# linjieli222/HERO

Measured on AMD Instinct MI355X. Metric: videos/sec training step, HERO-base TVR-shaped batch, higher is better.
Workload: dtype bf16; 1 GPU; configs[1]: HERO-base TVR finetune micro-step (train-tvr-8gpu.json shapes: 32 videos x 60 frames, 15 subs x (4 frames + 20 tokens), 15-token query; vfeat 4352; fwd + VSM loss + bwd, all-reduce/clip/AdamW every 2nd micro-step); global_batch=32, parallelism=dp1, grad_accum=2, launch=hipGraph replay, input=one batch resident in HBM

## Files before the change

hero_amd/_lib.py:

```python
import ctypes as C
import os

import torch

_HERE = os.path.dirname(os.path.abspath(__file__))
LIB_PATH = os.environ.get("HERO_HIP_LIB") or os.path.join(_HERE, "libhero_hip.so")

ABI_VERSION = 3
F32, BF16 = 0, 1
LAYOUT_K, LAYOUT_O = 0, 1
ACT_NONE, ACT_GELU, ACT_RELU, ACT_GELU_BWD, ACT_RELU_BWD, ACT_GELU_DG, ACT_MUL_AUX = 0, 1, 2, 3, 4, 5, 6

EXPORTS = [
    "hero_last_error", "hero_abi_version", "hero_abi_struct_count", "hero_abi_struct_bytes", "hero_gemm", "hero_gemm_splits", "hero_fold_slabs", "hero_wgrad_group", "hero_wgrad_batch_plan", "hero_wgrad_batch", "hero_prof_enable", "hero_prof_read", "hero_probe_mfma", "hero_probe_hbm", "hero_gemm_force_config", "hero_layernorm_fwd",
    "hero_layernorm_bwd_workspace_bytes", "hero_layernorm_bwd", "hero_colsum_workspace_bytes",
    "hero_colsum", "hero_colsum_multi", "hero_colsum_multi_workspace_bytes", "hero_layernorm_bwd_blocks", "hero_attention_fwd", "hero_attention_bwd", "hero_attention_max_len", "hero_attention_max_packed_len", "hero_attention_stats_ok", "hero_attention_force_ppw",
    "hero_gather_rows", "hero_inverse_first", "hero_csr_gather_sum", "hero_scatter_add_rows", "hero_segment_sort_workspace_bytes", "hero_scatter_add_sorted_workspace_bytes", "hero_segment_sort", "hero_scatter_add_sorted", "hero_cast", "hero_transpose_cast", "hero_copy_multi",
    "hero_relu_bwd", "hero_gelu_bwd", "hero_add", "hero_sumsq", "hero_adamw", "hero_adamw_multi", "hero_adamw_multi_chunk",
    "hero_query_pool_fwd", "hero_query_pool_bwd", "hero_rownorm_fwd", "hero_rownorm_bwd", "hero_score_max_fwd",
    "hero_score_max_bwd", "hero_rank_loss", "hero_sums_scaled", "hero_st_ed_fwd", "hero_st_ed_bwd", "hero_st_ed_bwd_workspace_bytes",
    "hero_cross_entropy_fwd", "hero_cross_entropy_bwd",
    "hero_collate_subs", "hero_collate_clip_mask", "hero_collate_frame_map", "hero_collate_gather_feats", "hero_derive_multi",
    "hero_comm_available", "hero_comm_unique_id", "hero_comm_init", "hero_comm_destroy", "hero_comm_rank", "hero_comm_world",
    "hero_comm_allreduce_buckets", "hero_comm_broadcast", "hero_comm_allgather", "hero_comm_allgather_var",
]


class Dropout(C.Structure):
    _fields_ = [("seed_ptr", C.c_void_p), ("site", C.c_uint64),
                ("threshold16", C.c_uint32), ("scale", C.c_float)]


class GemmEpilogue(C.Structure):
    _fields_ = [("bias", C.c_void_p), ("residual", C.c_void_p), ("aux", C.c_void_p),
                ("act", C.c_int), ("out_f32", C.c_int), ("beta", C.c_float),
                ("split_k", C.c_int), ("dropout", Dropout), ("colsum", C.c_void_p), ("colsum_partial", C.c_int), ("pad_", C.c_int), ("split_stride", C.c_longlong)]


class CrossEntropy(C.Structure):
    _fields_ = [("logits", C.c_void_p), ("labels", C.c_void_p), ("loss", C.c_void_p), ("lse", C.c_void_p),
                ("dloss", C.c_void_p), ("dlogits", C.c_void_p), ("rows", C.c_int), ("cols", C.c_int),
                ("ld", C.c_int), ("dtype", C.c_int), ("inv_temp", C.c_float), ("ignore_index", C.c_int64)]


class Derive(C.Structure):
    _fields_ = [("src", C.c_void_p), ("dst", C.c_void_p), ("n", C.c_int64), ("mode", C.c_int), ("p0", C.c_int),
                ("p1", C.c_int), ("p2", C.c_int)]
# ... 121 lines not shown
    global _lib
    if _lib is None:
        if not os.path.exists(LIB_PATH):
            raise RuntimeError(
                "hero_amd: %s is missing. Build it with `python -m hero_amd.build` "
                "(needs hipcc; cross-compiles for gfx950 without a GPU). There is no fallback "
                "path." % LIB_PATH)
        L = C.CDLL(LIB_PATH)
        L.hero_last_error.restype = C.c_char_p
        have = L.hero_abi_version()
        if have != ABI_VERSION:
            raise RuntimeError("hero_amd: %s reports ABI version %d, this binding was written against %d (struct layouts "
                               "differ: rebuild with `python -m hero_amd.build --force`)" % (LIB_PATH, have, ABI_VERSION))
        L.hero_abi_struct_bytes.argtypes = [C.c_int]
        if L.hero_abi_struct_count() != len(ABI_STRUCTS):
            raise RuntimeError("hero_amd: %s declares %d ABI structs, this binding mirrors %d" % (LIB_PATH, L.hero_abi_struct_count(), len(ABI_STRUCTS)))
        bad = [(st.__name__, C.sizeof(st), L.hero_abi_struct_bytes(i)) for i, st in enumerate(ABI_STRUCTS)
               if C.sizeof(st) != L.hero_abi_struct_bytes(i)]
        if bad:
            raise RuntimeError("hero_amd: struct layouts differ from %s (name, binding bytes, library bytes): %s" % (LIB_PATH, bad))
        L.hero_layernorm_bwd_workspace_bytes.restype = C.c_size_t
        L.hero_colsum_workspace_bytes.restype = C.c_size_t
        L.hero_colsum_multi_workspace_bytes.restype = C.c_size_t
        L.hero_colsum_multi_workspace_bytes.argtypes = [C.POINTER(Colsum), C.c_int]
        L.hero_colsum_multi.argtypes = [C.POINTER(Colsum), C.c_int, C.c_void_p, C.c_void_p]
        L.hero_layernorm_bwd_blocks.argtypes = [C.c_int]
        L.hero_gemm.argtypes = [C.c_void_p, C.c_void_p, C.c_void_p] + [C.c_int] * 9 + [
            C.POINTER(GemmEpilogue), C.c_void_p]
        L.hero_gemm_splits.argtypes = [C.c_int, C.c_int, C.c_int]
        L.hero_fold_slabs.argtypes = [C.c_void_p, C.c_int, C.c_size_t, C.c_void_p, C.c_size_t, C.c_int, C.c_void_p]
        L.hero_wgrad_group.argtypes = [C.POINTER(WgradProblem), C.c_int, C.c_int, C.c_int, C.c_void_p]
        L.hero_wgrad_batch_plan.argtypes = [C.POINTER(WgradProblem), C.c_int, C.c_int, C.c_void_p, C.c_int]
        L.hero_wgrad_batch.argtypes = [C.POINTER(WgradProblem), C.c_int, C.c_int, C.c_int, C.c_void_p, C.c_int, C.c_void_p]
        L.hero_prof_enable.argtypes = [C.c_int]
        L.hero_prof_read.argtypes = [C.c_int, C.POINTER(C.c_double), C.POINTER(C.c_double),
                                     C.POINTER(C.c_longlong)]
        L.hero_probe_mfma.argtypes = [C.c_void_p, C.c_size_t, C.POINTER(C.c_double), C.POINTER(C.c_double), C.c_void_p]
        L.hero_probe_hbm.argtypes = [C.c_void_p, C.c_void_p, C.c_size_t, C.POINTER(C.c_double), C.POINTER(C.c_double), C.c_void_p]
        L.hero_layernorm_fwd.argtypes = [C.POINTER(LnFwd), C.c_void_p]
        L.hero_layernorm_bwd.argtypes = [C.POINTER(LnBwd), C.c_void_p]
        L.hero_layernorm_bwd_workspace_bytes.argtypes = [C.c_int, C.c_int]
        L.hero_colsum_workspace_bytes.argtypes = [C.c_int, C.c_int]
        L.hero_colsum.argtypes = [C.c_void_p, C.c_void_p, C.c_int, C.c_int, C.c_int, C.c_int,
                                  C.c_float, C.c_void_p, C.c_void_p]
        L.hero_attention_fwd.argtypes = [C.POINTER(Attn), C.c_void_p]
        L.hero_attention_bwd.argtypes = [C.POINTER(Attn), C.c_void_p]
        L.hero_attention_stats_ok.argtypes = [C.c_int, C.c_int]
        L.hero_attention_force_ppw.argtypes = [C.c_int]
        L.hero_attention_max_len.argtypes = [C.c_int, C.c_int]
        L.hero_attention_max_packed_len.argtypes = [C.c_int]
        L.hero_gather_rows.argtypes = [C.c_void_p, C.c_void_p, C.c_void_p, C.c_void_p,
                                       C.c_int, C.c_int, C.c_int, C.c_void_p]
        L.hero_inverse_first.argtypes = [C.c_void_p, C.c_int, C.c_void_p, C.c_int, C.c_int, C.c_void_p]
        L.hero_csr_gather_sum.argtypes = [C.c_void_p, C.c_void_p, C.c_void_p, C.c_void_p,
                                          C.c_int, C.c_int, C.c_int, C.c_void_p]
        L.hero_scatter_add_rows.argtypes = [C.c_void_p, C.c_void_p, C.c_void_p, C.c_void_p,
                                            C.c_int, C.c_int, C.c_int, C.c_int, C.c_int, C.c_void_p]
        L.hero_segment_sort_workspace_bytes.argtypes = [C.c_int]
        L.hero_segment_sort_workspace_bytes.restype = C.c_size_t
        L.hero_segment_sort.argtypes = [C.c_void_p, C.c_int, C.c_int, C.c_int, C.c_void_p, C.c_void_p, C.c_void_p]
        L.hero_scatter_add_sorted_workspace_bytes.argtypes = [C.c_int, C.c_int]
        L.hero_scatter_add_sorted_workspace_bytes.restype = C.c_size_t
        L.hero_scatter_add_sorted.argtypes = [C.c_void_p, C.c_void_p, C.c_void_p, C.c_void_p, C.c_int, C.c_int, C.c_int, C.c_int,
                                              C.c_void_p, C.c_void_p]
        L.hero_st_ed_bwd_workspace_bytes.argtypes = [C.c_int]
        L.hero_st_ed_bwd_workspace_bytes.restype = C.c_size_t
# ... 74 lines not shown
```

hero_amd/csrc/gemm_ws.hip:

```cpp
#include <stdlib.h>
#include <type_traits>

#include "gemm_ws_common.h"

namespace hero {
namespace ws {

template <int TM, int TN, bool TR, int EK>
__global__ __launch_bounds__(512) __attribute__((amdgpu_waves_per_eu(2, 2))) void gemm_ws_kernel(WsArgs g) {
  typedef Geo<TM, TN> G;
  extern __shared__ __attribute__((aligned(16))) char smem[];
  const int lane = threadIdx.x & 63;
  const int wave = __builtin_amdgcn_readfirstlane(threadIdx.x >> 6);
  const int nwg = gridDim.x;
  int wg;
  {
    const int bid = blockIdx.x, q = nwg >> 3, r = nwg & 7, xcd = bid & 7, loc = bid >> 3;
    wg = (xcd < r ? xcd * (q + 1) : r * (q + 1) + (xcd - r) * q) + loc;
  }

  if (wave >= 4) {
    Loader<G, TR> ld(g, smem, wg, nwg, wave - 4, lane);
    constexpr int AHEAD = (G::NSG - 2) * G::PW;
    bool more = ld.issue();
#pragma unroll
    for (int k = 0; k < G::NSG - 2; ++k) more = ld.issue();
    if (more) wait_vm<AHEAD>(); else wait_vm<0>();
    __builtin_amdgcn_s_barrier();
    unsigned slot = 0;
    int item_no = 0;
    for (int cit = wg; cit < g.nwork; cit += nwg, ++item_no) {
      const Item ic = item_coord<G>(g, cit);
      WS_T(item_no, 0, wave, lane);
// ... 351 lines not shown
      __builtin_amdgcn_s_barrier();
      __builtin_amdgcn_sched_barrier(0);
      ldf(a0, b0, nxt, 0);
      mma(a1, b1);
      WS_INTERLEAVE(TM * TN, 2 * (TM + TN));
      __builtin_amdgcn_sched_barrier(0);
    }
    pos += sg.nk;
    WS_T(seg_no, 1, wave, lane);
#ifdef HERO_WS_TRACE
    if (blockIdx.x == 0 && lane == 0 && seg_no < 4) g_ws_trace[(seg_no * 16 + 3) * 8 + wave] = (unsigned long long)sg.nk;
#endif
    const WsgProb& P = g.p[sg.prob];
#pragma unroll
    for (int i = 0; i < TM; ++i)
#pragma unroll
      for (int j = 0; j < TN; ++j) {
        const int gn = sg.n0 + brow0 + j * 32 + (lane & 31);
#pragma unroll
        for (int r = 0; r < 16; ++r) {
          const int gm = sg.m0 + arow0 + i * 32 + (r & 3) + 8 * (r >> 2) + 4 * (lane >> 5);
          if (gm < P.M && gn < P.N) atomicAdd(P.C + (size_t)gm * P.ldc + gn, acc[i][j][r]);
        }
      }
    WS_T(seg_no, 14, wave, lane);
  }
}

struct WsbProb {
  const bf16_t* A;
  const bf16_t* B;
  float* C;
  float* colsum;
  int M, N, lda, ldb, ldc, pad_;
};
struct WsbItem { int prob, m0, n0, k0, nk, order, nslices, flag; };
struct WsbArgs {
  const WsbItem* items;
  int* flags;
  int rounds, K, nprob, pad_;
  WsbProb p[HERO_WGRAD_BATCH_MAX];
};

template <typename G, bool COMPUTE>
__device__ __forceinline__ void epilogue_acc(const WsbProb& P, const WsbItem& it, int* flags, char* smem, unsigned slot,
                                             f32x16_t (*acc)[G::TN], int wave, int lane, bool want_cs = false) {
  constexpr int TM = G::TM, TN = G::TN, BN = G::BN, RPP = G::RPP, C8 = G::C8, RPI = G::RPI, ITERS = G::ITERS;
  char* st = smem + slot;
  int tid = threadIdx.x;
  asm volatile("" : "+v"(tid));
  lane = tid & 63;
  wave = __builtin_amdgcn_readfirstlane(tid >> 6);
  const int c8 = tid % C8, r0 = tid / C8;
  const int gn = it.n0 + c8 * 8;
  const bool col_ok = r0 < RPI && gn < P.N;
  const int wm = wave >> 1, wn = wave & 1, l31 = lane & 31, half = lane >> 5;
  const bool plain = it.nslices == 1;
  constexpr bool SPLIT = (RPP == 64 && G::PASSES == TM);
  auto tile_row = [](int p, int row) { return SPLIT ? (row >> 5) * (TM * 32) + p * 32 + (row & 31) : p * RPP + row; };
  const __amdgpu_buffer_rsrc_t rc = __builtin_amdgcn_make_buffer_rsrc(P.C, 0, 0x7ffffff0, 0x00020000);
  if (!plain && it.order > 0) {
    if (lane == 0)
      while (__hip_atomic_load(flags + it.flag, __ATOMIC_RELAXED, __HIP_MEMORY_SCOPE_AGENT) != it.order) __builtin_amdgcn_s_sleep(8);
  }
#pragma unroll
  for (int p = 0; p < G::PASSES; ++p) {
    u32x4_t old0[ITERS], old1[ITERS];
    unsigned voff[ITERS];
    if (plain) {
#pragma unroll
      for (int i = 0; i < ITERS; ++i) {
        const int row = r0 + i * RPI;
        const int gm = it.m0 + tile_row(p, row);
        const bool ok = col_ok && row < RPP && gm < P.M;
// ... 98 lines not shown
    wg = (xcd < r ? xcd * (q + 1) : r * (q + 1) + (xcd - r) * q) + loc;
  }
  auto next_round = [&](int r) {
    while (r < g.rounds && g.items[(size_t)r * nwg + wg].nk == 0) ++r;
    return r;
  };

  if (wave >= 4) {
    const int w = wave - 4;
    constexpr int CA = G::BM / 8, CB = G::BN / 8;
    int lr = next_round(0), ik = 0, lnk = 0;
    unsigned goa[G::PA], gob[G::PB];
    const char* pa = nullptr;
    const char* pb = nullptr;
    unsigned long long ra_left = 0, rb_left = 0;
    unsigned sa = 0, sb = 0, fill = 0;
    auto setup = [&]() {
      const WsbItem it = g.items[(size_t)lr * nwg + wg];
      const WsbProb& P = g.p[it.prob];
      lnk = it.nk;
#pragma unroll
      for (int i = 0; i < G::PA; ++i) {
        const int id = (w * G::PA + i) * 64 + lane, row = id / CA, c = (id % CA) ^ swz_o<G::BM * 2>(row);
        goa[i] = (unsigned)row * (unsigned)P.lda * 2u + (c << 4);
      }
#pragma unroll
      for (int i = 0; i < G::PB; ++i) {
        const int id = (w * G::PB + i) * 64 + lane, row = id / CB, c = (id % CB) ^ swz_o<G::BN * 2>(row);
        gob[i] = (unsigned)row * (unsigned)P.ldb * 2u + (c << 4);
      }
      const int kb = it.k0 * 64;
      pa = reinterpret_cast<const char*>(P.A + (size_t)kb * P.lda + it.m0);
      pb = reinterpret_cast<const char*>(P.B + (size_t)kb * P.ldb + it.n0);
      ra_left = ((unsigned long long)(g.K - kb) * P.lda - it.m0) * 2;
      rb_left = ((unsigned long long)(g.K - kb) * P.ldb - it.n0) * 2;
      sa = 64u * (unsigned)P.lda * 2u;
      sb = 64u * (unsigned)P.ldb * 2u;
    };
    if (lr < g.rounds) setup();
    auto issue = [&]() -> bool {
      if (lr >= g.rounds) return false;
      char* buf = smem + fill;
      const __amdgpu_buffer_rsrc_t ra = __builtin_amdgcn_make_buffer_rsrc(const_cast<char*>(pa), 0, (unsigned)(ra_left < 0xfffffff0ull ? ra_left : 0xfffffff0ull), 0x00020000);
      const __amdgpu_buffer_rsrc_t rb = __builtin_amdgcn_make_buffer_rsrc(const_cast<char*>(pb), 0, (unsigned)(rb_left < 0xfffffff0ull ? rb_left : 0xfffffff0ull), 0x00020000);
#ifndef HERO_WSB_NOLOADS
#pragma unroll
      for (int i = 0; i < G::PA; ++i)
        __builtin_amdgcn_raw_ptr_buffer_load_lds(ra, HERO_LDS_PTR(buf + (w * G::PA + i) * 1024), 16, goa[i], 0, 0, HERO_WS_LOAD_AUX_A);
#pragma unroll
      for (int i = 0; i < G::PB; ++i)
        __builtin_amdgcn_raw_ptr_buffer_load_lds(rb, HERO_LDS_PTR(buf + G::A_BYTES + (w * G::PB + i) * 1024), 16, gob[i], 0, 0, HERO_WS_LOAD_AUX_B);
#else
      (void)ra; (void)rb; (void)buf;
#endif
      fill += G::STAGE;
      if (fill == NS * G::STAGE) fill = 0;
      if (++ik == lnk) {
        ik = 0;
        lr = next_round(lr + 1);
        if (lr < g.rounds) setup();
      } else {
        pa += sa; pb += sb;
        ra_left = ra_left > sa ? ra_left - sa : 0ull;
        rb_left = rb_left > sb ? rb_left - sb : 0ull;
      }
      return true;
    };
    issue();
// ... 324 lines not shown
    P.M = q.M; P.N = q.N; P.lda = q.ld_dy; P.ldb = q.ld_x; P.ldc = q.ld_dw;
    P.tiles_n = (q.N + G::BN - 1) / G::BN;
    P.tile0 = tiles;
    tiles += ((q.M + G::BM - 1) / G::BM) * P.tiles_n;
  }
  const int ksteps = (K + 63) / 64;
  const int cus = num_cus();
  if (ok && (long long)tiles * ksteps >= 8LL * cus) {
    for (int i = n; i < 4; ++i) g.p[i] = g.p[0];
    g.nprob = n; g.K = K; g.ksteps = ksteps; g.total_tiles = tiles;
    HERO_ENSURE_LDS(&gemm_wsg_kernel, G::LDS, "gemm_wsg_kernel");
    double flops = 0.0;
    for (int i = 0; i < n; ++i) flops += 2.0 * probs[i].M * (double)probs[i].N * K;
    void* tok = gemm_prof_begin(9, s);
    hipLaunchKernelGGL(gemm_wsg_kernel, dim3(cus), dim3(512), G::LDS, s, g);
    gemm_prof_end(tok, flops, s);
    return check_launch("hero_wgrad_group");
  }
  for (int i = 0; i < n; ++i) {
    const HeroWgradProblem& q = probs[i];
    HeroGemmEpilogue e = {};
    e.out_f32 = 1; e.beta = 1.f; e.split_k = q.split_hint > 0 ? q.split_hint : 1; e.dropout.scale = 1.f;
    const int rc = hero_gemm(q.dy, q.x, q.dw, q.M, q.N, K, q.ld_dy, q.ld_x, q.ld_dw, HERO_LAYOUT_O, HERO_LAYOUT_O, dtype, &e, stream);
    if (rc) return rc;
  }
  return HERO_OK;
}

namespace hero {
namespace ws {
__device__ int g_wsb_flags[512];
constexpr int PLAN_MAGIC = 0x57534232;
constexpr int PLAN_HDR = 8;
}
}

extern "C" int hero_wgrad_batch_plan(const HeroWgradProblem* probs, int n, int K, int32_t* plan, int capacity_words) {
  using namespace hero;
  using namespace hero::ws;
  typedef Geo<3, 3> G;
  HERO_REQUIRE(probs && n >= 1 && n <= HERO_WGRAD_BATCH_MAX, "hero_wgrad_batch_plan: 1..%d problems", HERO_WGRAD_BATCH_MAX);
  HERO_REQUIRE(K >= 1, "hero_wgrad_batch_plan: K = %d", K);
  const int nwg = num_cus(), ksteps = (K + 63) / 64;
  if (nwg % 8 != 0 || ksteps < 8) return 0;
  struct T3 { int prob, mt, nt; };
  std::vector<T3> tiles;
  for (int i = 0; i < n; ++i) {
    HERO_REQUIRE(probs[i].M > 0 && probs[i].N > 0 && probs[i].M % 8 == 0 && probs[i].N % 8 == 0, "hero_wgrad_batch_plan: bad problem %d", i);
    const int tm = (probs[i].M + G::BM - 1) / G::BM, tn = (probs[i].N + G::BN - 1) / G::BN;
    const int per = nwg / 8;
    int pm = tm < 8 ? tm : 8;
    int pn = per / pm > 0 ? per / pm : 1;
    if (pn > tn) { pn = tn; pm = per / pn < tm ? per / pn : tm; if (pm < 1) pm = 1; }
    for (int bm = 0; bm < tm; bm += pm)
      for (int bn = 0; bn < tn; bn += pn)
        for (int mi = bm; mi < bm + pm && mi < tm; ++mi)
          for (int ni = bn; ni < bn + pn && ni < tn; ++ni) tiles.push_back({i, mi, ni});
  }
  const int T = (int)tiles.size();
  const int full = T / nwg, rem = T % nwg;
  struct Piece { int slot, round, tile, k0, nk, order, nslices; };
  std::vector<Piece> pieces;
  int tail_rounds = rem ? 1 : 0, S = 1;
  const int per_xcd_cap = nwg / 8, per_xcd = rem ? (rem + 7) / 8 : 0;
  if (rem) {
    HERO_REQUIRE(per_xcd <= 512 / 8, "hero_wgrad_batch_plan: flag capacity");
    for (int xcd = 0; xcd * per_xcd < rem; ++xcd) {
      const int t0 = xcd * per_xcd, p = (rem - t0 < per_xcd) ? rem - t0 : per_xcd, c = per_xcd_cap;
      int Sx = c / p;
      while (Sx > 1 && ksteps / Sx < 4) --Sx;
      if (Sx > 8) Sx = 8;
      auto cost_us = [&](int sl) { return (double)((ksteps + sl - 1) / sl) * 1.17 + (sl == 1 ? 8.0 : 9.0 + 16.0 * sl); };
      while (Sx > 1 && cost_us(Sx - 1) <= cost_us(Sx)) --Sx;
      const int L = c - Sx * p;
      const int E = 6;
      int q = (int)(((long long)p * ksteps + (long long)(p - L) * E + c - 1) / c);
      int r = ksteps - Sx * q;
      if (L == 0 || Sx != c / p || ksteps < 128 || r * 8 < ksteps) { r = 0; q = ksteps; }
      if (xcd == 0) S = Sx;
      std::vector<std::vector<Piece>> of_tile(p);
      int slot = Sx * p, fillq = 0, rnd = 0;
      for (int t = 0; t < p && r > 0; ++t) {
        int left = r;
        std::vector<Piece> mine;
        while (left > 0) {
          int room = q - fillq;
          if (slot >= c - 1) room = left;
          else if (room < 2 || (room < left && left - room < 2)) {
            if (room < 2) { ++slot; fillq = 0; rnd = 0; continue; }
            room = left;
// ... 16 lines not shown
        }
        for (Piece& pc : of_tile[t]) {
          pc.nslices = (int)of_tile[t].size();
          pc.slot += xcd * per_xcd_cap;
          pc.tile = t0 + t;
          if (pc.round + 1 > tail_rounds) tail_rounds = pc.round + 1;
          pieces.push_back(pc);
        }
      }
    }
  }
  const int rounds = full + tail_rounds;
  const int words = PLAN_HDR + rounds * nwg * 8;
  HERO_REQUIRE(plan && capacity_words >= words, "hero_wgrad_batch_plan: needs %d words, capacity %d", words, capacity_words);
  for (int i = PLAN_HDR; i < words; ++i) plan[i] = 0;
  auto item = [&](int r, int w) { return plan + PLAN_HDR + ((size_t)r * nwg + w) * 8; };
  for (int r = 0; r < full; ++r)
    for (int w = 0; w < nwg; ++w) {
      const T3& t = tiles[(size_t)r * nwg + w];
      int32_t* q = item(r, w);
      q[0] = t.prob; q[1] = t.mt * G::BM; q[2] = t.nt * G::BN; q[3] = 0; q[4] = ksteps; q[5] = 0; q[6] = 1; q[7] = 0;
    }
  for (const Piece& pc : pieces) {
    const T3& t = tiles[(size_t)full * nwg + pc.tile];
    int32_t* q = item(full + pc.round, pc.slot);
    HERO_REQUIRE(q[4] == 0, "hero_wgrad_batch_plan: internal error (slot used twice)");
    q[0] = t.prob; q[1] = t.mt * G::BM; q[2] = t.nt * G::BN; q[3] = pc.k0; q[4] = pc.nk; q[5] = pc.order; q[6] = pc.nslices;
    q[7] = (pc.slot / per_xcd_cap) * (512 / 8) + (pc.tile % per_xcd);
  }
  plan[0] = PLAN_MAGIC; plan[1] = nwg; plan[2] = rounds; plan[3] = rounds * nwg; plan[4] = n; plan[5] = K; plan[6] = T; plan[7] = S;
  return words;
}

extern "C" int hero_wgrad_batch(const HeroWgradProblem* probs, int n, int K, int dtype, const int32_t* plan_dev, int plan_words,
                                hero_stream_t stream) {
  using namespace hero;
  using namespace hero::ws;
  typedef Geo<3, 3> G;
  HERO_REQUIRE(probs && n >= 1 && n <= HERO_WGRAD_BATCH_MAX, "hero_wgrad_batch: 1..%d problems", HERO_WGRAD_BATCH_MAX);
  HERO_REQUIRE(dtype == HERO_BF16, "hero_wgrad_batch: bf16 only (dtype %d)", dtype);
  HERO_REQUIRE(plan_dev && plan_words > PLAN_HDR && (plan_words - PLAN_HDR) % (8 * num_cus()) == 0,
               "hero_wgrad_batch: the plan (%d words) was not made for this device (%d workgroups)", plan_words, num_cus());
  HERO_REQUIRE(((uintptr_t)plan_dev & 15) == 0, "hero_wgrad_batch: plan_dev must be 16-byte aligned");
  hipStream_t s = static_cast<hipStream_t>(stream);
  WsbArgs g;
  double flops = 0.0;
  for (int i = 0; i < n; ++i) {
    const HeroWgradProblem& q = probs[i];
    HERO_REQUIRE(q.dy && q.x && q.dw && q.M > 0 && q.N > 0 && q.M % 8 == 0 && q.N % 8 == 0 && q.ld_dy % 8 == 0 && q.ld_x % 8 == 0 &&
                     q.ld_dw % 4 == 0 && (((uintptr_t)q.dy | (uintptr_t)q.x | (uintptr_t)q.dw) & 15) == 0 &&
                     (size_t)64 * q.ld_dy * 2 < 0x7fffffffull && (size_t)64 * q.ld_x * 2 < 0x7fffffffull &&
                     (size_t)q.M * q.ld_dw * 4 < 0x7ffffff0ull,
                 "hero_wgrad_batch: problem %d is unaligned / too large", i);
    WsbProb& P = g.p[i];
    P.A = static_cast<const bf16_t*>(q.dy); P.B = static_cast<const bf16_t*>(q.x); P.C = q.dw;
    P.M = q.M; P.N = q.N; P.lda = q.ld_dy; P.ldb = q.ld_x; P.ldc = q.ld_dw; P.pad_ = 0;
    P.colsum = q.dbias;
    flops += 2.0 * q.M * (double)q.N * K;
  }
  for (int i = n; i < HERO_WGRAD_BATCH_MAX; ++i) g.p[i] = g.p[0];
  g.items = reinterpret_cast<const WsbItem*>(plan_dev + PLAN_HDR);
  g.rounds = (plan_words - PLAN_HDR) / (8 * num_cus());
  g.K = K; g.nprob = n; g.pad_ = 0;
  static int* flags_of[64] = {};
  int dev = 0;
  (void)hipGetDevice(&dev);
  HERO_REQUIRE(dev >= 0 && dev < 64, "hero_wgrad_batch: device %d", dev);
  if (!flags_of[dev]) HERO_REQUIRE(hipGetSymbolAddress(reinterpret_cast<void**>(&flags_of[dev]), HIP_SYMBOL(hero::ws::g_wsb_flags)) == hipSuccess,
                                   "hero_wgrad_batch: flag storage");
  g.flags = flags_of[dev];
  HERO_ENSURE_LDS(&gemm_wsb_kernel, G::LDS, "gemm_wsb_kernel");
  void* tok = gemm_prof_begin(9, s);
  hipLaunchKernelGGL(gemm_wsb_kernel, dim3(num_cus()), dim3(512), G::LDS, s, g);
  gemm_prof_end(tok, flops, s);
  return check_launch("hero_wgrad_batch");
}
```

hero_amd/functional.py:

```python
import ctypes as C
import math
import os
import weakref

import numpy as np
import torch

from . import _lib as L

_COMPUTE_DTYPE = torch.bfloat16


def set_compute_dtype(dtype):
    global _COMPUTE_DTYPE
    if dtype not in (torch.float32, torch.bfloat16):
        raise ValueError("compute dtype must be torch.float32 or torch.bfloat16")
    _COMPUTE_DTYPE = dtype


def compute_dtype():
    return _COMPUTE_DTYPE


class _Rng:
# ... 272 lines not shown
        k_gemm(dy2, Wt, slabs, M, K, n1, N, N, K, L.LAYOUT_K, L.LAYOUT_K, L.BF16, out_f32=True)
    if n1 < N:
        k_gemm(L.ptr(dy2) + 2 * n1, L.ptr(Wt) + 2 * n1, L.ptr(slabs) + 4 * n_main * stride, M, K, N - n1, N, N, K,
               L.LAYOUT_K, L.LAYOUT_K, L.BF16, out_f32=True)
    out = torch.empty((M, K), dtype=torch.bfloat16, device=dy2.device)
    L.check(L.lib().hero_fold_slabs(L.ptr(slabs), slabs.shape[0], stride, L.ptr(out), stride, L.BF16, L.stream()))
    return out


def _split_for(n_out, n_in, rows, bk):
    tiles = ((n_out + 127) // 128) * ((n_in + 127) // 128)
    ktiles = max(1, -(-rows // bk))
    flops = 2.0 * n_out * n_in * rows
    out_bytes = 4.0 * n_out * n_in
    best, best_t = 1, None
    for s in range(1, 17):
        if s > 1 and ktiles // s < 4:
            break
        blocks = tiles * s
        rounds = -(-blocks // 512)
        last = blocks - (rounds - 1) * 512
        t = flops / blocks * ((rounds - 1) / 1.83e12 + (1 / 2.7e12 if last <= 256 else 1 / 1.83e12))
        if s > 1:
            t += out_bytes * s / 2.0e12
        if best_t is None or t < best_t:
            best, best_t = s, t
    return best


_WQ = []
_WQ_TASK = [-1]
GROUP_WGRADS = [True]
WGRAD_BATCH = [32]
WGRAD_DBIAS_RIDE = [True]
WGRAD_RIDE_MAX_ROWS = [1 << 30]
B1_EPILOGUE = [False]
B1_PARTIALS = [True]
WGRAD_QUEUE_BYTES = [int(os.environ.get("HERO_WGRAD_QUEUE_MB", "4096")) << 20]
_WQ_BYTES = [0]
_WPLANS = {}
_WPLANS_PINNED = set()


def _wgrad_queue_full(device):
    if _WQ_BYTES[0] <= WGRAD_QUEUE_BYTES[0]:
        return False
    hard = _WQ_HARD.get(device.index)
    if hard is None:
        env = os.environ.get("HERO_WGRAD_QUEUE_HARD_MB")
        hard = (int(env) << 20) if env else max(2 * WGRAD_QUEUE_BYTES[0], int(0.15 * torch.cuda.get_device_properties(device).total_memory))
        _WQ_HARD[device.index] = hard
    if _WQ_BYTES[0] > hard:
        return True
    tiles = sum(-(-e[4] // 192) * -(-e[1].shape[1] // 192) for e in _WQ)
    full, rem = divmod(tiles, 256)
    if rem == 0:
        return True
    p = -(-rem // 8)
    slices = max(1, min(32 // p, 8))
    return tiles / 256.0 >= 0.9 * (full + (1.4 if slices > 1 else 1.0) / slices)


_WQ_HARD = {}


def _wgrad_limit():
    return 4 if (WGRAD_BATCH[0] <= 4 or SINK.wants_overlap()) else min(WGRAD_BATCH[0], 32)


def _wgrad_plan(probs, n, rows, device):
    key = (rows, device.index, tuple((probs[i].M, probs[i].N) for i in range(n)))
    hit = _WPLANS.get(key, False)
    if hit is False:
        buf = np.zeros(8 + 8 * 512 * 16, dtype=np.int32)
        words = L.lib().hero_wgrad_batch_plan(probs, n, rows, buf.ctypes.data, buf.size)
        if words < 0:
            L.check(words)
        hit = (torch.from_numpy(buf[:words].copy()).to(device), words) if words > 0 else None
        if len(_WPLANS) > 256:
            for k in [k for k in _WPLANS if k not in _WPLANS_PINNED][:128]:
                del _WPLANS[k]
        _WPLANS[key] = hit
    if hit is not None and torch.cuda.is_current_stream_capturing():
        _WPLANS_PINNED.add(key)
    return hit


_CB_TASK = [-1]


def _ensure_flush_callback(task):
    if _CB_TASK[0] != task:
        _CB_TASK[0] = task
        torch.autograd.Variable._execution_engine.queue_callback(deferred_flush)


def deferred_flush():
    _CB_TASK[0] = -1
    wgrad_flush()
    colsum_flush()


_CQ = []
_CQ_TASK = [-1]


def _colsum_defer_ok():
    return GROUP_WGRADS[0] and not SINK.wants_overlap() and torch._C._current_graph_task_id() != -1
# ... 7 lines not shown
    _ensure_flush_callback(task)
    _CQ.append(((keep, dst_rows), L.Colsum(src_ptr, L.ptr(dst), rows, cols, ld, dtype, 1.0, row_cols, L.ptr(dst_rows)), dst, on_done))
    if len(_CQ) >= 64:
        colsum_flush()


def colsum_flush():
    while _CQ:
        part, seen = [], []
        while _CQ and len(part) < 64:
            lo = _CQ[0][1].dst
            hi = lo + 4 * _CQ[0][2].numel()
            if any(lo < b and a < hi for a, b in seen):
                break
            seen.append((lo, hi))
            part.append(_CQ.pop(0))
        n = len(part)
        probs = (L.Colsum * n)(*[e[1] for e in part])
        need = L.lib().hero_colsum_multi_workspace_bytes(probs, n) // 4
        ws = _workspace(max(need, 1), part[0][2].device, slot="colsum_multi")
        L.check(L.lib().hero_colsum_multi(probs, n, L.ptr(ws), L.stream()))
        for e in part:
            if e[3] is not None:
                e[3]()


def wgrad_flush():
    _WQ_BYTES[0] = 0
    while _WQ:
        rows, dtype = _WQ[0][0].shape[0], _WQ[0][0].dtype
        dst_key = lambda e: (e[2].data_ptr(), e[6].data_ptr() if e[6] is not None else None)
        seen_w, seen_b = {_WQ[0][2].data_ptr()}, {dst_key(_WQ[0])[1]} - {None}
        n = 1
        while n < len(_WQ) and n < 32 and _WQ[n][0].shape[0] == rows and _WQ[n][0].dtype == dtype:
            kw, kb = dst_key(_WQ[n])
            if kw in seen_w or (kb is not None and kb in seen_b):
                break
            seen_w.add(kw)
            if kb is not None:
                seen_b.add(kb)
            n += 1
        group, rest = _WQ[:n], _WQ[n:]
        del _WQ[:]
        _WQ.extend(rest)
        probs = (L.WgradProblem * n)()
        for i, (dy2, x2, out, col0, N, _, _, _) in enumerate(group):
            K = x2.shape[1]
            probs[i] = L.WgradProblem(L.ptr(dy2) + col0 * dy2.element_size(), L.ptr(x2), L.ptr(out), N, K,
                                      dy2.shape[1], K, K, _split_for(N, K, rows, 64 if dtype == torch.bfloat16 else 32), None)
        plan = _wgrad_plan(probs, n, rows, group[0][0].device) if dtype == torch.bfloat16 else None
        if plan is not None:
            ride = WGRAD_DBIAS_RIDE[0] and rows <= WGRAD_RIDE_MAX_ROWS[0]
            for i, e in enumerate(group):
                probs[i].dbias = L.ptr(e[6]) if ride else None
                if not ride and e[6] is not None:
                    k_colsum(e[0], out=e[6], beta=1.0, col0=e[3], ncols=e[4], on_done=lambda: None)
            L.check(L.lib().hero_wgrad_batch(probs, n, rows, L.BF16, L.ptr(plan[0]), plan[1], L.stream()))
            for e in group:
                if e[6] is not None and e[7] is not None:
                    e[7]()
        else:
            for g0 in range(0, n, 4):
                sub = (L.WgradProblem * min(4, n - g0))(*[probs[i] for i in range(g0, min(g0 + 4, n))])
                L.check(L.lib().hero_wgrad_group(sub, len(sub), rows, L.dt(group[0][0]), L.stream()))
            for dy2, _, _, col0, N, _, dbias, dbias_done in group:
                if dbias is not None:
                    k_colsum(dy2, out=dbias, beta=1.0, col0=col0, ncols=N, on_done=dbias_done or (lambda: None))
        for e in group:
            if e[5] is not None:
                e[5]()


def k_wgrad(dy2, x2, out=None, beta=0.0, col0=0, ncols=None, on_done=None, dbias=None, dbias_done=None):
    M, ld = dy2.shape
    N = ld - col0 if ncols is None else ncols
    K = x2.shape[1]
    if (out is not None and beta == 1.0 and GROUP_WGRADS[0] and out.is_contiguous() and dy2.is_contiguous()
            and x2.is_contiguous() and torch._C._current_graph_task_id() != -1):
        task = torch._C._current_graph_task_id()
        if _WQ and _WQ_TASK[0] != task:
            del _WQ[:]
            _WQ_BYTES[0] = 0
        if _WQ and (_WQ[0][0].shape[0] != M or _WQ[0][0].dtype != dy2.dtype):
            wgrad_flush()
        if not _WQ:
            _WQ_TASK[0] = task
        _ensure_flush_callback(task)
        _WQ.append((dy2, x2, out, col0, N, on_done, dbias, dbias_done))
        _WQ_BYTES[0] += dy2.numel() * dy2.element_size()
        if len(_WQ) >= _wgrad_limit() or _wgrad_queue_full(dy2.device):
            wgrad_flush()
        return out
    if dbias is not None:
        k_colsum(dy2, out=dbias, beta=1.0, col0=col0, ncols=N, on_done=dbias_done or (lambda: None))
    if out is None:
        out = torch.empty((N, K), dtype=torch.float32, device=dy2.device)
    split = _split_for(N, K, M, 64 if dy2.dtype == torch.bfloat16 else 32)
    a = L.ptr(dy2) + col0 * dy2.element_size()
    k_gemm(a, x2, out, N, K, M, ld, K, K, L.LAYOUT_O, L.LAYOUT_O, L.dt(dy2), out_f32=True,
           beta=beta, split_k=split)
    if on_done is not None:
        on_done()
    return out


_WS = {}


def _workspace(n_floats, device, slot=""):
    key = (device.type, device.index, slot)
    t = _WS.get(key)
    if t is None or t.numel() < n_floats:
        t = torch.empty((max(n_floats, 1 << 20),), dtype=torch.float32, device=device)
        _WS[key] = t
    return t

# ... 913 lines not shown
```

include/hero_hip.h:

```cpp
#ifndef HERO_HIP_H_
#define HERO_HIP_H_

#include <stddef.h>
#include <stdint.h>

#ifdef __cplusplus
extern "C" {
#endif

typedef void* hero_stream_t;

enum { HERO_F32 = 0, HERO_BF16 = 1 };
enum { HERO_OK = 0, HERO_ERR_ARG = -1, HERO_ERR_LAUNCH = -2, HERO_ERR_UNSUPPORTED = -3 };

const char* hero_last_error(void);
#define HERO_ABI_VERSION 3
int hero_abi_version(void);
enum { HERO_STRUCT_DROPOUT = 0, HERO_STRUCT_GEMM_EPILOGUE, HERO_STRUCT_WGRAD_PROBLEM, HERO_STRUCT_LN_FWD, HERO_STRUCT_LN_BWD,
       HERO_STRUCT_COLSUM, HERO_STRUCT_ATTN, HERO_STRUCT_ADAMW, HERO_STRUCT_TENSOR_DESC, HERO_STRUCT_ADAMW_GROUP,
       HERO_STRUCT_ADAMW_MULTI, HERO_STRUCT_COPY_DESC, HERO_STRUCT_QUERY_POOL, HERO_STRUCT_ROW_NORM, HERO_STRUCT_SCORE_MAX,
       HERO_STRUCT_RANK_LOSS, HERO_STRUCT_ST_ED, HERO_STRUCT_CROSS_ENTROPY, HERO_STRUCT_DERIVE, HERO_STRUCT_COMM_BUCKET,
       HERO_STRUCT_COUNT_ };
int hero_abi_struct_count(void);
int hero_abi_struct_bytes(int which);
// ... 18 lines not shown
typedef struct HeroGemmEpilogue {
  const float* bias;
  const void* residual;
  void* aux;
  int act;
  int out_f32;
  float beta;
  int split_k;
  HeroDropout dropout;
  float* colsum;
  int colsum_partial;
  int pad_;
  long long split_stride;
} HeroGemmEpilogue;

int hero_gemm(const void* A, const void* B, void* C, int M, int N, int K, int lda, int ldb, int ldc,
              int a_layout, int b_layout, int dtype, const HeroGemmEpilogue* epi, hero_stream_t stream);
int hero_gemm_splits(int K, int split_k, int dtype);
int hero_fold_slabs(const float* slabs, int n_slabs, size_t stride, void* out, size_t n, int out_dtype, hero_stream_t stream);

typedef struct HeroWgradProblem {
  const void* dy;
  const void* x;
  float* dw;
  int M, N, ld_dy, ld_x, ld_dw;
  int split_hint;
  float* dbias;
} HeroWgradProblem;
int hero_wgrad_group(const HeroWgradProblem* probs, int n, int K, int dtype, hero_stream_t stream);
#define HERO_WGRAD_BATCH_MAX 32
int hero_wgrad_batch_plan(const HeroWgradProblem* probs, int n, int K, int32_t* plan, int capacity_words);
int hero_wgrad_batch(const HeroWgradProblem* probs, int n, int K, int dtype, const int32_t* plan_dev, int plan_words,
                     hero_stream_t stream);
int hero_gemm_force_config(int cfg);
int hero_prof_enable(int on);
int hero_prof_read(int slot, double* total_ms, double* total_flops, long long* launches);

int hero_probe_mfma(void* scratch, size_t scratch_bytes, double* tflops, double* ghz, hero_stream_t stream);
int hero_probe_hbm(const void* src, void* dst, size_t bytes, double* copy_gbps, double* read_gbps, hero_stream_t stream);

typedef struct HeroLnFwd {
  const void* x;
  const float* tab[3];
  const int32_t* idx[3];
  const float* gamma;
  const float* beta;
  void* y;
  void* pre;
  float* mean;
  float* rstd;
  int rows, cols;
  float eps;
  int x_dtype, y_dtype;
  HeroDropout dropout;
} HeroLnFwd;
int hero_layernorm_fwd(const HeroLnFwd* a, hero_stream_t stream);

typedef struct HeroLnBwd {
  const void* x;
  const void* dy;
  const float* gamma;
  const float* mean;
  const float* rstd;
  void* dx;
  void* dx_dropped;
  float* dgamma;
// ... 269 lines not shown
```

Baseline: 5194 videos/s.

## Batch weight-gradient GEMMs with mixed row counts into one persistent launch

Gives each batched wgrad problem its own K (row count), so queued weight-gradient GEMMs with different token counts (video frames, subtitles, queries) can share one persistent work-stealing launch. The old code flushed whenever the row count changed. A new host planner greedily load-balances whole tiles across CUs by estimated cost. It optionally reuses the split-K plan for the longest-K problems when that lowers the estimated makespan. The cost is a larger per-launch argument struct (64 problems), a queue that holds more pending work, and a heuristic cost model that may produce imbalanced schedules.

```diff
diff --git a/hero_amd/_lib.py b/hero_amd/_lib.py
--- a/hero_amd/_lib.py
+++ b/hero_amd/_lib.py
@@ -12,7 +12,7 @@
 ACT_NONE, ACT_GELU, ACT_RELU, ACT_GELU_BWD, ACT_RELU_BWD, ACT_GELU_DG, ACT_MUL_AUX = 0, 1, 2, 3, 4, 5, 6
 
 EXPORTS = [
-    "hero_last_error", "hero_abi_version", "hero_abi_struct_count", "hero_abi_struct_bytes", "hero_gemm", "hero_gemm_splits", "hero_fold_slabs", "hero_wgrad_group", "hero_wgrad_batch_plan", "hero_wgrad_batch", "hero_prof_enable", "hero_prof_read", "hero_probe_mfma", "hero_probe_hbm", "hero_gemm_force_config", "hero_layernorm_fwd",
+    "hero_last_error", "hero_abi_version", "hero_abi_struct_count", "hero_abi_struct_bytes", "hero_gemm", "hero_gemm_splits", "hero_fold_slabs", "hero_wgrad_group", "hero_wgrad_batch_plan", "hero_wgrad_batch", "hero_wgrad_batch_plan_rows", "hero_wgrad_batch_rows", "hero_prof_enable", "hero_prof_read", "hero_probe_mfma", "hero_probe_hbm", "hero_gemm_force_config", "hero_layernorm_fwd",
     "hero_layernorm_bwd_workspace_bytes", "hero_layernorm_bwd", "hero_colsum_workspace_bytes",
     "hero_colsum", "hero_colsum_multi", "hero_colsum_multi_workspace_bytes", "hero_layernorm_bwd_blocks", "hero_attention_fwd", "hero_attention_bwd", "hero_attention_max_len", "hero_attention_max_packed_len", "hero_attention_stats_ok", "hero_attention_force_ppw",
     "hero_gather_rows", "hero_inverse_first", "hero_csr_gather_sum", "hero_scatter_add_rows", "hero_segment_sort_workspace_bytes", "hero_scatter_add_sorted_workspace_bytes", "hero_segment_sort", "hero_scatter_add_sorted", "hero_cast", "hero_transpose_cast", "hero_copy_multi",
@@ -200,6 +200,8 @@
         L.hero_wgrad_group.argtypes = [C.POINTER(WgradProblem), C.c_int, C.c_int, C.c_int, C.c_void_p]
         L.hero_wgrad_batch_plan.argtypes = [C.POINTER(WgradProblem), C.c_int, C.c_int, C.c_void_p, C.c_int]
         L.hero_wgrad_batch.argtypes = [C.POINTER(WgradProblem), C.c_int, C.c_int, C.c_int, C.c_void_p, C.c_int, C.c_void_p]
+        L.hero_wgrad_batch_plan_rows.argtypes = [C.POINTER(WgradProblem), C.c_int, C.POINTER(C.c_int), C.c_void_p, C.c_int]
+        L.hero_wgrad_batch_rows.argtypes = [C.POINTER(WgradProblem), C.c_int, C.POINTER(C.c_int), C.c_int, C.c_void_p, C.c_int, C.c_void_p]
         L.hero_prof_enable.argtypes = [C.c_int]
         L.hero_prof_read.argtypes = [C.c_int, C.POINTER(C.c_double), C.POINTER(C.c_double),
                                      C.POINTER(C.c_longlong)]
diff --git a/hero_amd/csrc/gemm_ws.hip b/hero_amd/csrc/gemm_ws.hip
--- a/hero_amd/csrc/gemm_ws.hip
+++ b/hero_amd/csrc/gemm_ws.hip
@@ -1,4 +1,5 @@
 #include <stdlib.h>
+#include <algorithm>
 #include <type_traits>
 
 #include "gemm_ws_common.h"
@@ -416,14 +417,14 @@
   const bf16_t* B;
   float* C;
   float* colsum;
-  int M, N, lda, ldb, ldc, pad_;
+  int M, N, lda, ldb, ldc, K;
 };
 struct WsbItem { int prob, m0, n0, k0, nk, order, nslices, flag; };
 struct WsbArgs {
   const WsbItem* items;
   int* flags;
-  int rounds, K, nprob, pad_;
-  WsbProb p[HERO_WGRAD_BATCH_MAX];
+  int rounds, nprob;
+  WsbProb p[HERO_WGRAD_ROWS_MAX];
 };
 
 template <typename G, bool COMPUTE>
@@ -588,8 +589,8 @@
       const int kb = it.k0 * 64;
       pa = reinterpret_cast<const char*>(P.A + (size_t)kb * P.lda + it.m0);
       pb = reinterpret_cast<const char*>(P.B + (size_t)kb * P.ldb + it.n0);
-      ra_left = ((unsigned long long)(g.K - kb) * P.lda - it.m0) * 2;
-      rb_left = ((unsigned long long)(g.K - kb) * P.ldb - it.n0) * 2;
+      ra_left = ((unsigned long long)(P.K - kb) * P.lda - it.m0) * 2;
+      rb_left = ((unsigned long long)(P.K - kb) * P.ldb - it.n0) * 2;
       sa = 64u * (unsigned)P.lda * 2u;
       sb = 64u * (unsigned)P.ldb * 2u;
     };
@@ -980,6 +981,20 @@
 __device__ int g_wsb_flags[512];
 constexpr int PLAN_MAGIC = 0x57534232;
 constexpr int PLAN_HDR = 8;
+
+struct T3 { int prob, mt, nt; };
+static void patch_tiles(const HeroWgradProblem& q, int prob, int nwg, std::vector<T3>& tiles) {
+  typedef Geo<3, 3> G;
+  const int tm = (q.M + G::BM - 1) / G::BM, tn = (q.N + G::BN - 1) / G::BN;
+  const int per = nwg / 8;
+  int pm = tm < 8 ? tm : 8;
+  int pn = per / pm > 0 ? per / pm : 1;
+  if (pn > tn) { pn = tn; pm = per / pn < tm ? per / pn : tm; if (pm < 1) pm = 1; }
+  for (int bm = 0; bm < tm; bm += pm)
+    for (int bn = 0; bn < tn; bn += pn)
+      for (int mi = bm; mi < bm + pm && mi < tm; ++mi)
+        for (int ni = bn; ni < bn + pn && ni < tn; ++ni) tiles.push_back({prob, mi, ni});
+}
 }
 }
 
@@ -991,19 +1006,10 @@
   HERO_REQUIRE(K >= 1, "hero_wgrad_batch_plan: K = %d", K);
   const int nwg = num_cus(), ksteps = (K + 63) / 64;
   if (nwg % 8 != 0 || ksteps < 8) return 0;
-  struct T3 { int prob, mt, nt; };
   std::vector<T3> tiles;
   for (int i = 0; i < n; ++i) {
     HERO_REQUIRE(probs[i].M > 0 && probs[i].N > 0 && probs[i].M % 8 == 0 && probs[i].N % 8 == 0, "hero_wgrad_batch_plan: bad problem %d", i);
-    const int tm = (probs[i].M + G::BM - 1) / G::BM, tn = (probs[i].N + G::BN - 1) / G::BN;
-    const int per = nwg / 8;
-    int pm = tm < 8 ? tm : 8;
-    int pn = per / pm > 0 ? per / pm : 1;
-    if (pn > tn) { pn = tn; pm = per / pn < tm ? per / pn : tm; if (pm < 1) pm = 1; }
-    for (int bm = 0; bm < tm; bm += pm)
-      for (int bn = 0; bn < tn; bn += pn)
-        for (int mi = bm; mi < bm + pm && mi < tm; ++mi)
-          for (int ni = bn; ni < bn + pn && ni < tn; ++ni) tiles.push_back({i, mi, ni});
+    patch_tiles(probs[i], i, nwg, tiles);
   }
   const int T = (int)tiles.size();
   const int full = T / nwg, rem = T % nwg;
@@ -1086,12 +1092,129 @@
   return words;
 }
 
-extern "C" int hero_wgrad_batch(const HeroWgradProblem* probs, int n, int K, int dtype, const int32_t* plan_dev, int plan_words,
-                                hero_stream_t stream) {
+extern "C" int hero_wgrad_batch_plan_rows(const HeroWgradProblem* probs, int n, const int* rows, int32_t* plan, int capacity_words) {
   using namespace hero;
   using namespace hero::ws;
   typedef Geo<3, 3> G;
+  HERO_REQUIRE(probs && rows && n >= 1 && n <= HERO_WGRAD_ROWS_MAX, "hero_wgrad_batch_plan_rows: 1..%d problems", HERO_WGRAD_ROWS_MAX);
+  const int nwg = num_cus();
+  bool same = true;
+  int rmax = 0, T = 0;
+  for (int i = 0; i < n; ++i) {
+    HERO_REQUIRE(rows[i] >= 1 && probs[i].M > 0 && probs[i].N > 0 && probs[i].M % 8 == 0 && probs[i].N % 8 == 0,
+                 "hero_wgrad_batch_plan_rows: bad problem %d", i);
+    same = same && rows[i] == rows[0];
+    rmax = rows[i] > rmax ? rows[i] : rmax;
+    T += ((probs[i].M + G::BM - 1) / G::BM) * ((probs[i].N + G::BN - 1) / G::BN);
+  }
+  auto deliver = [&](const std::vector<int32_t>& v, int words) -> int {
+    if (!plan) return words;
+    HERO_REQUIRE(capacity_words >= words, "hero_wgrad_batch_plan_rows: needs %d words, capacity %d", words, capacity_words);
+    for (int i = 0; i < words; ++i) plan[i] = v[i];
+    return words;
+  };
+  auto equal_plan = [&](const std::vector<int>& idx, int K, std::vector<int32_t>& v) -> int {
+    std::vector<HeroWgradProblem> sub;
+    int t = 0;
+    for (int i : idx) { sub.push_back(probs[i]); t += ((probs[i].M + G::BM - 1) / G::BM) * ((probs[i].N + G::BN - 1) / G::BN); }
+    v.assign(PLAN_HDR + (size_t)(t / nwg + 40) * nwg * 8, 0);
+    return hero_wgrad_batch_plan(sub.data(), (int)sub.size(), K, v.data(), (int)v.size());
+  };
+  if (same && n <= HERO_WGRAD_BATCH_MAX) {
+    std::vector<int> all(n);
+    for (int i = 0; i < n; ++i) all[i] = i;
+    std::vector<int32_t> v;
+    const int words = equal_plan(all, rows[0], v);
+    return words > 0 ? deliver(v, words) : words;
+  }
+  if (nwg % 8 != 0 || (rmax + 63) / 64 < 8) return 0;
+  std::vector<int> order(n);
+  for (int i = 0; i < n; ++i) order[i] = i;
+  auto ks = [&](int i) { return (rows[i] + 63) / 64; };
+  std::stable_sort(order.begin(), order.end(), [&](int a, int b) { return ks(a) > ks(b); });
+  struct It { int prob, m0, n0, k0, nk, order, nslices, flag; };
+  auto build = [&](bool sliced, std::vector<std::vector<It>>& lists, long long& makespan, int& S) -> bool {
+    lists.assign(nwg, {});
+    std::vector<long long> load(nwg, 0);
+    std::vector<char> placed(n, 0);
+    S = 1;
+    if (sliced) {
+      std::vector<int> idx;
+      for (int i = 0; i < n; ++i) if (rows[i] == rmax) idx.push_back(i);
+      if ((int)idx.size() > HERO_WGRAD_BATCH_MAX) return false;
+      std::vector<int32_t> v;
+      const int words = equal_plan(idx, rmax, v);
+      if (words <= PLAN_HDR || v[7] <= 1) return false;
+      S = v[7];
+      const int rounds = v[2];
+      for (int r = 0; r < rounds; ++r)
+        for (int w = 0; w < nwg; ++w) {
+          const int32_t* q = v.data() + PLAN_HDR + ((size_t)r * nwg + w) * 8;
+          if (q[4] == 0) continue;
+          lists[w].push_back({idx[q[0]], q[1], q[2], q[3], q[4], q[5], q[6], q[7]});
+          load[w] += q[6] == 1 ? q[4] * 117LL + 800 : q[4] * 117LL + 900 + 1600LL * q[6];
+        }
+      for (int i : idx) placed[i] = 1;
+    }
+    std::vector<T3> tiles;
+    for (int i : order) {
+      if (placed[i]) continue;
+      tiles.clear();
+      patch_tiles(probs[i], i, nwg, tiles);
+      for (const T3& t : tiles) {
+        int w = 0;
+        for (int x = 1; x < nwg; ++x) if (load[x] < load[w]) w = x;
+        lists[w].push_back({i, t.mt * G::BM, t.nt * G::BN, 0, ks(i), 0, 1, 0});
+        load[w] += ks(i) * 117LL + 800;
+      }
+    }
+    makespan = 0;
+    for (int w = 0; w < nwg; ++w) makespan = load[w] > makespan ? load[w] : makespan;
+    return true;
+  };
+  std::vector<std::vector<It>> whole, cut;
+  long long t_whole = 0, t_cut = 0;
+  int S = 1, S_cut = 1;
+  build(false, whole, t_whole, S);
+  const bool use_cut = build(true, cut, t_cut, S_cut) && t_cut < t_whole;
+  const std::vector<std::vector<It>>& lists = use_cut ? cut : whole;
+  int rounds = 0;
+  for (int w = 0; w < nwg; ++w) rounds = (int)lists[w].size() > rounds ? (int)lists[w].size() : rounds;
+  const int words = PLAN_HDR + rounds * nwg * 8;
+  std::vector<int32_t> v(words, 0);
+  for (int w = 0; w < nwg; ++w)
+    for (int r = 0; r < (int)lists[w].size(); ++r) {
+      const It& it = lists[w][r];
+      int32_t* q = v.data() + PLAN_HDR + ((size_t)r * nwg + w) * 8;
+      q[0] = it.prob; q[1] = it.m0; q[2] = it.n0; q[3] = it.k0; q[4] = it.nk; q[5] = it.order; q[6] = it.nslices; q[7] = it.flag;
+    }
+  v[0] = PLAN_MAGIC; v[1] = nwg; v[2] = rounds; v[3] = rounds * nwg; v[4] = n; v[5] = 0; v[6] = T; v[7] = use_cut ? S_cut : 1;
+  return deliver(v, words);
+}
+
+static int wsb_launch(const char* who, const HeroWgradProblem* probs, int n, const int* rows, int K, int dtype, const int32_t* plan_dev,
+                      int plan_words, hero_stream_t stream);
+
+extern "C" int hero_wgrad_batch(const HeroWgradProblem* probs, int n, int K, int dtype, const int32_t* plan_dev, int plan_words,
+                                hero_stream_t stream) {
   HERO_REQUIRE(probs && n >= 1 && n <= HERO_WGRAD_BATCH_MAX, "hero_wgrad_batch: 1..%d problems", HERO_WGRAD_BATCH_MAX);
+  HERO_REQUIRE(K >= 1, "hero_wgrad_batch: K = %d", K);
+  return wsb_launch("hero_wgrad_batch", probs, n, nullptr, K, dtype, plan_dev, plan_words, stream);
+}
+
+extern "C" int hero_wgrad_batch_rows(const HeroWgradProblem* probs, int n, const int* rows, int dtype, const int32_t* plan_dev,
+                                     int plan_words, hero_stream_t stream) {
+  HERO_REQUIRE(probs && rows && n >= 1 && n <= HERO_WGRAD_ROWS_MAX, "hero_wgrad_batch_rows: 1..%d problems", HERO_WGRAD_ROWS_MAX);
+  for (int i = 0; i < n; ++i) HERO_REQUIRE(rows[i] >= 1, "hero_wgrad_batch_rows: rows[%d] = %d", i, rows[i]);
+  return wsb_launch("hero_wgrad_batch_rows", probs, n, rows, 0, dtype, plan_dev, plan_words, stream);
+}
+
+static int wsb_launch(const char* who, const HeroWgradProblem* probs, int n, const int* rows, int K, int dtype, const int32_t* plan_dev,
+                      int plan_words, hero_stream_t stream) {
+  using namespace hero;
+  using namespace hero::ws;
+  typedef Geo<3, 3> G;
+  (void)who;
   HERO_REQUIRE(dtype == HERO_BF16, "hero_wgrad_batch: bf16 only (dtype %d)", dtype);
   HERO_REQUIRE(plan_dev && plan_words > PLAN_HDR && (plan_words - PLAN_HDR) % (8 * num_cus()) == 0,
                "hero_wgrad_batch: the plan (%d words) was not made for this device (%d workgroups)", plan_words, num_cus());
@@ -1108,14 +1231,14 @@
                  "hero_wgrad_batch: problem %d is unaligned / too large", i);
     WsbProb& P = g.p[i];
     P.A = static_cast<const bf16_t*>(q.dy); P.B = static_cast<const bf16_t*>(q.x); P.C = q.dw;
-    P.M = q.M; P.N = q.N; P.lda = q.ld_dy; P.ldb = q.ld_x; P.ldc = q.ld_dw; P.pad_ = 0;
+    P.M = q.M; P.N = q.N; P.lda = q.ld_dy; P.ldb = q.ld_x; P.ldc = q.ld_dw; P.K = rows ? rows[i] : K;
     P.colsum = q.dbias;
-    flops += 2.0 * q.M * (double)q.N * K;
-  }
-  for (int i = n; i < HERO_WGRAD_BATCH_MAX; ++i) g.p[i] = g.p[0];
+    flops += 2.0 * q.M * (double)q.N * P.K;
+  }
+  for (int i = n; i < HERO_WGRAD_ROWS_MAX; ++i) g.p[i] = g.p[0];
   g.items = reinterpret_cast<const WsbItem*>(plan_dev + PLAN_HDR);
   g.rounds = (plan_words - PLAN_HDR) / (8 * num_cus());
-  g.K = K; g.nprob = n; g.pad_ = 0;
+  g.nprob = n;
   static int* flags_of[64] = {};
   int dev = 0;
   (void)hipGetDevice(&dev);
diff --git a/hero_amd/functional.py b/hero_amd/functional.py
--- a/hero_amd/functional.py
+++ b/hero_amd/functional.py
@@ -328,6 +328,8 @@
 _WQ_TASK = [-1]
 GROUP_WGRADS = [True]
 WGRAD_BATCH = [32]
+WGRAD_MIXED_ROWS = [True]
+WGRAD_ROWS_MAX = 64
 WGRAD_DBIAS_RIDE = [True]
 WGRAD_RIDE_MAX_ROWS = [1 << 30]
 B1_EPILOGUE = [False]
@@ -361,15 +363,20 @@
 
 
 def _wgrad_limit():
-    return 4 if (WGRAD_BATCH[0] <= 4 or SINK.wants_overlap()) else min(WGRAD_BATCH[0], 32)
+    if WGRAD_BATCH[0] <= 4 or SINK.wants_overlap():
+        return 4
+    return WGRAD_ROWS_MAX if WGRAD_MIXED_ROWS[0] else min(WGRAD_BATCH[0], 32)
 
 
 def _wgrad_plan(probs, n, rows, device):
     key = (rows, device.index, tuple((probs[i].M, probs[i].N) for i in range(n)))
     hit = _WPLANS.get(key, False)
     if hit is False:
-        buf = np.zeros(8 + 8 * 512 * 16, dtype=np.int32)
-        words = L.lib().hero_wgrad_batch_plan(probs, n, rows, buf.ctypes.data, buf.size)
+        rows_c = (C.c_int * n)(*rows)
+        words = L.lib().hero_wgrad_batch_plan_rows(probs, n, rows_c, None, 0)
+        if words > 0:
+            buf = np.zeros(words, dtype=np.int32)
+            words = L.lib().hero_wgrad_batch_plan_rows(probs, n, rows_c, buf.ctypes.data, buf.size)
         if words < 0:
             L.check(words)
         hit = (torch.from_numpy(buf[:words].copy()).to(device), words) if words > 0 else None
@@ -443,7 +450,9 @@
         dst_key = lambda e: (e[2].data_ptr(), e[6].data_ptr() if e[6] is not None else None)
         seen_w, seen_b = {_WQ[0][2].data_ptr()}, {dst_key(_WQ[0])[1]} - {None}
         n = 1
-        while n < len(_WQ) and n < 32 and _WQ[n][0].shape[0] == rows and _WQ[n][0].dtype == dtype:
+        mixed = WGRAD_MIXED_ROWS[0] and dtype == torch.bfloat16
+        cap = WGRAD_ROWS_MAX if mixed else 32
+        while n < len(_WQ) and n < cap and (mixed or _WQ[n][0].shape[0] == rows) and _WQ[n][0].dtype == dtype:
             kw, kb = dst_key(_WQ[n])
             if kw in seen_w or (kb is not None and kb in seen_b):
                 break
@@ -455,25 +464,31 @@
         del _WQ[:]
         _WQ.extend(rest)
         probs = (L.WgradProblem * n)()
+        rows_of = tuple(e[0].shape[0] for e in group)
         for i, (dy2, x2, out, col0, N, _, _, _) in enumerate(group):
             K = x2.shape[1]
             probs[i] = L.WgradProblem(L.ptr(dy2) + col0 * dy2.element_size(), L.ptr(x2), L.ptr(out), N, K,
-                                      dy2.shape[1], K, K, _split_for(N, K, rows, 64 if dtype == torch.bfloat16 else 32), None)
-        plan = _wgrad_plan(probs, n, rows, group[0][0].device) if dtype == torch.bfloat16 else None
+                                      dy2.shape[1], K, K, _split_for(N, K, rows_of[i], 64 if dtype == torch.bfloat16 else 32), None)
+        plan = _wgrad_plan(probs, n, rows_of, group[0][0].device) if dtype == torch.bfloat16 else None
         if plan is not None:
-            ride = WGRAD_DBIAS_RIDE[0] and rows <= WGRAD_RIDE_MAX_ROWS[0]
             for i, e in enumerate(group):
+                ride = WGRAD_DBIAS_RIDE[0] and rows_of[i] <= WGRAD_RIDE_MAX_ROWS[0]
                 probs[i].dbias = L.ptr(e[6]) if ride else None
                 if not ride and e[6] is not None:
                     k_colsum(e[0], out=e[6], beta=1.0, col0=e[3], ncols=e[4], on_done=lambda: None)
-            L.check(L.lib().hero_wgrad_batch(probs, n, rows, L.BF16, L.ptr(plan[0]), plan[1], L.stream()))
+            L.check(L.lib().hero_wgrad_batch_rows(probs, n, (C.c_int * n)(*rows_of), L.BF16, L.ptr(plan[0]), plan[1], L.stream()))
             for e in group:
                 if e[6] is not None and e[7] is not None:
                     e[7]()
         else:
-            for g0 in range(0, n, 4):
-                sub = (L.WgradProblem * min(4, n - g0))(*[probs[i] for i in range(g0, min(g0 + 4, n))])
-                L.check(L.lib().hero_wgrad_group(sub, len(sub), rows, L.dt(group[0][0]), L.stream()))
+            g0 = 0
+            while g0 < n:
+                g1 = g0 + 1
+                while g1 < n and g1 - g0 < 4 and rows_of[g1] == rows_of[g0]:
+                    g1 += 1
+                sub = (L.WgradProblem * (g1 - g0))(*[probs[i] for i in range(g0, g1)])
+                L.check(L.lib().hero_wgrad_group(sub, len(sub), rows_of[g0], L.dt(group[0][0]), L.stream()))
+                g0 = g1
             for dy2, _, _, col0, N, _, dbias, dbias_done in group:
                 if dbias is not None:
                     k_colsum(dy2, out=dbias, beta=1.0, col0=col0, ncols=N, on_done=dbias_done or (lambda: None))
@@ -492,7 +507,9 @@
         if _WQ and _WQ_TASK[0] != task:
             del _WQ[:]
             _WQ_BYTES[0] = 0
-        if _WQ and (_WQ[0][0].shape[0] != M or _WQ[0][0].dtype != dy2.dtype):
+        mixed = (WGRAD_MIXED_ROWS[0] and dy2.dtype == torch.bfloat16 and not SINK.wants_overlap()
+                 and 2 * (_WQ_BYTES[0] + dy2.numel() * dy2.element_size()) <= WGRAD_QUEUE_BYTES[0])
+        if _WQ and (_WQ[0][0].dtype != dy2.dtype or (not mixed and _WQ[-1][0].shape[0] != M)):
             wgrad_flush()
         if not _WQ:
             _WQ_TASK[0] = task
diff --git a/include/hero_hip.h b/include/hero_hip.h
--- a/include/hero_hip.h
+++ b/include/hero_hip.h
@@ -74,6 +74,10 @@
 int hero_wgrad_batch_plan(const HeroWgradProblem* probs, int n, int K, int32_t* plan, int capacity_words);
 int hero_wgrad_batch(const HeroWgradProblem* probs, int n, int K, int dtype, const int32_t* plan_dev, int plan_words,
                      hero_stream_t stream);
+#define HERO_WGRAD_ROWS_MAX 64
+int hero_wgrad_batch_plan_rows(const HeroWgradProblem* probs, int n, const int* rows, int32_t* plan, int capacity_words);
+int hero_wgrad_batch_rows(const HeroWgradProblem* probs, int n, const int* rows, int dtype, const int32_t* plan_dev,
+                          int plan_words, hero_stream_t stream);
 int hero_gemm_force_config(int cfg);
 int hero_prof_enable(int on);
 int hero_prof_read(int slot, double* total_ms, double* total_flops, long long* launches);
```

Result: faster. 5270 videos/s (median of 6 runs) (+1.5%).
